# AIBluefisher/DAGSfM

Hardware: NVIDIA B200
Metric: image_pairs_verified_per_s (higher is better)
Workload: dtype f64 (verification) / u8 x u8 -> s32 exact (matching)

## Files before the change

### dagsfm_b200/csrc/verify_api.cu

```cuda
#include <cuda_runtime.h>

#include <algorithm>
#include <cstdio>
#include <cstdlib>
#include <cstring>
#include <vector>

#include "../../include/dagsfm_b200.h"
#include "common_host.h"
#include "verify_common.cuh"
#include "verify_multiple.h"

using namespace b2;

struct b2_verifier {
  int device = 0;
  int n_sm = 148;
  cudaStream_t stream = nullptr;
  int32_t n_images = 0;
  b2_camera* d_cams = nullptr;
  int64_t* d_img_off = nullptr;
  double* d_xy = nullptr;
  double* d_nxy = nullptr;
  int64_t n_pts_total = 0;
// ... 90 lines not shown
  }
  B2_CUDA(cudaMemsetAsync(v->d_err, 0, sizeof(int), s));
  VerifyArgs a;
  a.cams = v->d_cams;
  a.img_off = v->d_img_off;
  a.n_images = v->n_images;
  a.xy = (const double2*)v->d_xy;
  a.nxy = (const double2*)v->d_nxy;
  a.matches = matches;
  a.opt = *opt;
  a.inlier_out = inl;
  a.scratch = v->d_scratch;
  a.scratch_stride = stride;
  a.m_cap = m_cap;
  a.max_workers = blocks * wpb;
  a.work_counter = v->d_counter;
  a.state = (VerifyPairState*)v->d_state;
  a.masks = v->d_masks;
  a.mask_stride = std::max<int64_t>(max_span, 1);
  a.err = v->d_err;
  a.prof = nullptr;
  unsigned long long* d_prof = nullptr;
  if (getenv("B2_VERIFY_PROFILE")) {
    B2_CUDA(cudaMalloc(&d_prof, 8 * sizeof(unsigned long long)));
    B2_CUDA(cudaMemsetAsync(d_prof, 0, 8 * sizeof(unsigned long long), s));
    a.prof = d_prof;
  }
  B2_CUDA(cudaEventRecord(v->ev0, s));
  for (int64_t b = 0; b < n_batches; ++b) {
    const int64_t p0 = b * kStageBatch, p1 = std::min(n_pairs, p0 + kStageBatch);
    a.n_pairs = p1 - p0;
    a.pairs = pairs + 2 * p0;
    a.match_off = off + p0;
    a.seeds = seeds + p0;
    a.results = results + p0;
    a.mask_base = bound[(size_t)b];
    B2_CUDA(cudaMemsetAsync(v->d_counter, 0, 4 * sizeof(unsigned long long), s));
    B2_CUDA(launch_verify_pairs(a, v->n_sm, s));
    count_launches(4);
  }
  B2_CUDA(cudaEventRecord(v->ev1, s));
  count_launches(1);
  int err = 0;
  B2_CUDA(cudaMemcpyAsync(&err, v->d_err, sizeof(int), cudaMemcpyDeviceToHost, s));
  B2_CUDA(cudaStreamSynchronize(s));
  float ms = 0;
  B2_CUDA(cudaEventElapsedTime(&ms, v->ev0, v->ev1));
  v->last_kernel_s = ms * 1e-3;
  if (d_prof) {
    unsigned long long hp[8];
    cudaMemcpy(hp, d_prof, sizeof hp, cudaMemcpyDeviceToHost);
    cudaFree(d_prof);
    fprintf(stderr, "[b2 verify profile] warp-cycles: sample %.3g solve %.3g score %.3g lo %.3g | E %.3g F %.3g H %.3g T %.3g | kernel %.3f s\n",
            (double)hp[0], (double)hp[1], (double)hp[2], (double)hp[3], (double)hp[4], (double)hp[5], (double)hp[6], (double)hp[7], v->last_kernel_s);
  }
  if (err == 2) return set_error(B2_ERR_CUDA, "sampler FIFO exhausted inside one batch of trials (more than 256 raw draws)");
  if (err) return set_error(B2_ERR_INVALID, "pair references an image outside the store");
  return B2_OK;
}

int stage(b2_verifier* v, size_t bytes) {
  if (bytes <= v->stage_bytes) return B2_OK;
  if (v->d_stage) cudaFree(v->d_stage);
  v->d_stage = nullptr;
  v->stage_bytes = 0;
  B2_CUDA(cudaMalloc(&v->d_stage, bytes));
  v->stage_bytes = bytes;
  return B2_OK;
}

}

extern "C" {

void b2_two_view_default_options(b2_two_view_options* o) {
  if (!o) return;
  o->min_num_inliers = 15;
// ... 259 lines not shown
  if (n_pairs == 0) return check_options(opt);
  const int64_t total = match_offsets[n_pairs];
  if (total < 0 || (total > 0 && (!matches || !inlier_matches))) return set_error(B2_ERR_INVALID, "NULL match buffers");
  auto round = [&](int64_t na, const int64_t* ids, const int64_t* off, const uint32_t* m, const uint32_t* sd,
                   b2_two_view_result* res, uint32_t* inl) -> int {
    std::vector<uint32_t> pr((size_t)na * 2);
    for (int64_t k = 0; k < na; ++k) {
      pr[2 * k] = pairs[2 * ids[k]];
      pr[2 * k + 1] = pairs[2 * ids[k] + 1];
    }
    return b2_verify_pairs(v, na, pr.data(), off, m, opt, sd, res, inl);
  };
  return estimate_multiple(n_pairs, match_offsets, matches, seeds, multiple_ignore_watermark != 0, round, results,
                           inlier_matches);
}

int b2_score_models(b2_verifier* v, int32_t type, int32_t n, const double* xy1, const double* xy2, int32_t n_models,
                    const double* models, double max_residual, int32_t* counts, double* sums, uint8_t* masks) {
  if (!v || n < 0 || n_models < 0 || type < 0 || type > 3) return set_error(B2_ERR_INVALID, "bad argument");
  if (n_models == 0) return B2_OK;
  B2_CUDA(cudaSetDevice(v->device));
  auto al = [](size_t b) { return (b + 255) / 256 * 256; };
  const size_t bp = al((size_t)std::max(n, 1) * 16), bm = al((size_t)n_models * 72), bc = al((size_t)n_models * 4),
               bs = al((size_t)n_models * 8), bk = al((size_t)n_models * std::max(n, 1));
  B2_TRY(stage(v, 2 * bp + bm + bc + bs + bk));
  uint8_t* p = (uint8_t*)v->d_stage;
  double* d1 = (double*)p; p += bp;
  double* d2 = (double*)p; p += bp;
  double* dm = (double*)p; p += bm;
  int* dc = (int*)p; p += bc;
  double* ds = (double*)p; p += bs;
  uint8_t* dk = p;
  cudaStream_t s = v->stream;
  if (n > 0) {
    B2_CUDA(cudaMemcpyAsync(d1, xy1, (size_t)n * 16, cudaMemcpyHostToDevice, s));
    B2_CUDA(cudaMemcpyAsync(d2, xy2, (size_t)n * 16, cudaMemcpyHostToDevice, s));
  }
  B2_CUDA(cudaMemcpyAsync(dm, models, (size_t)n_models * 72, cudaMemcpyHostToDevice, s));
  B2_CUDA(launch_score_models(type, n, d1, d2, n_models, dm, max_residual, dc, ds, dk, s));
  count_launches(1);
  B2_CUDA(cudaMemcpyAsync(counts, dc, (size_t)n_models * 4, cudaMemcpyDeviceToHost, s));
  B2_CUDA(cudaMemcpyAsync(sums, ds, (size_t)n_models * 8, cudaMemcpyDeviceToHost, s));
  if (n > 0 && masks) B2_CUDA(cudaMemcpyAsync(masks, dk, (size_t)n_models * n, cudaMemcpyDeviceToHost, s));
  B2_CUDA(cudaStreamSynchronize(s));
  return B2_OK;
}

int b2_verify_debug_sample_stream(b2_verifier* v, uint32_t seed, int32_t total, int32_t k, int32_t n_trials,
                                  int32_t* out) {
  if (!v || !out || total < k || k < 1 || k > 8 || n_trials < 0) return set_error(B2_ERR_INVALID, "bad argument");
  B2_CUDA(cudaSetDevice(v->device));
  B2_TRY(stage(v, (size_t)total * 4 + (size_t)std::max(n_trials, 1) * k * 4 + 512));
  uint32_t* d_idx = (uint32_t*)v->d_stage;
  int* d_out = (int*)((uint8_t*)v->d_stage + ((size_t)total * 4 + 255) / 256 * 256);
  B2_CUDA(launch_debug_sample_stream(seed, total, k, n_trials, d_idx, d_out, v->stream));
  B2_CUDA(cudaMemcpyAsync(out, d_out, (size_t)n_trials * k * 4, cudaMemcpyDeviceToHost, v->stream));
  B2_CUDA(cudaStreamSynchronize(v->stream));
  return B2_OK;
}

int b2_verify_debug_solve(b2_verifier* v, int32_t type, int32_t n, const double* xy1, const double* xy2,
                          double* models_out, int32_t* n_models) {
// ... 36 lines not shown
```

### dagsfm_b200/csrc/verify_common.cuh

```cuda
#pragma once
#include <cuda_runtime.h>

#include <cstdint>

#include "../../include/dagsfm_b200.h"

namespace b2 {

enum { EST_E5 = 0, EST_F7 = 1, EST_H4 = 2, EST_T2 = 3 };
__host__ __device__ inline int min_samples(int t) { return t == EST_E5 ? 5 : t == EST_F7 ? 7 : t == EST_H4 ? 4 : 1; }
__host__ __device__ inline int local_min_samples(int t) { return t == EST_E5 ? 5 : t == EST_F7 ? 8 : t == EST_H4 ? 4 : 1; }

struct VerifyRansacReport {
  int32_t success, num_inliers;
  long long num_trials;
  double model[9];
};
struct VerifyPairState {
  uint32_t mt[624];
  uint32_t ring[256];
  uint32_t mti, w, r, pad;
  VerifyRansacReport report[3];
};

// ... 4 lines not shown
  const double2* xy;
  const double2* nxy;
  int64_t n_pairs;
  const uint32_t* pairs;
  const int64_t* match_off;
  const uint32_t* matches;
  const uint32_t* seeds;
  b2_two_view_options opt;
  b2_two_view_result* results;
  uint32_t* inlier_out;
  uint8_t* scratch;
  size_t scratch_stride;
  int32_t m_cap;
  int32_t max_workers;
  unsigned long long* work_counter;
  VerifyPairState* state;
  uint8_t* masks;
  int64_t mask_stride, mask_base;
  int* err;
  unsigned long long* prof;
};

size_t verify_scratch_stride(int m_cap);
int verify_warps_per_block();
int verify_blocks_per_sm();
cudaError_t launch_normalize_points(const b2_camera* cams, const int64_t* img_off, int n_images, const double* xy,
                                    double* nxy, int64_t n_total, cudaStream_t s);
cudaError_t launch_verify_pairs(const VerifyArgs& a, int n_sm, cudaStream_t s);
cudaError_t launch_relative_pose(const b2_camera* cams, const int64_t* img_off, int n_images, const double* nxy,
                                 int64_t n_pairs, const uint32_t* pairs, const int64_t* match_off,
                                 const b2_two_view_result* results, const uint32_t* inliers, b2_relative_pose* poses,
                                 double* angles, int* err, int n_sm, cudaStream_t s);
cudaError_t launch_score_models(int type, int n, const double* p1, const double* p2, int n_models, const double* models,
                                double max_res, int* counts, double* sums, uint8_t* masks, cudaStream_t s);
cudaError_t launch_debug_sample_stream(uint32_t seed, int total, int k, int n_trials, uint32_t* idx, int* out,
                                       cudaStream_t s);
cudaError_t launch_debug_solve(int type, int n, const double* p1, const double* p2, double* G, uint32_t* inl,
                               double* models, int* n_models, cudaStream_t s);

}
```

### dagsfm_b200/csrc/verify_kernel.cu

```cuda
#include <cuda_runtime.h>

#include <cfloat>
#include <cstdint>
#include <algorithm>
#include <cstdlib>
#include <cstring>

#include "../../include/dagsfm_b200.h"
#include "verify_common.cuh"
#include "verify_solvers.cuh"
#include "camera_models.cuh"

namespace b2 {
namespace vf {

constexpr unsigned kFull = 0xffffffffu;
constexpr int kWarpsPerBlock = 8;
constexpr int kThreads = 32 * kWarpsPerBlock;
using LaneView = View<1>;

constexpr int kIdxSmem = 2048;
struct WarpShared {
  double V[81];
  double R[81];
  double sig[9];
  uint32_t mt[624];
  uint32_t ring[256];
  uint16_t idx16[kIdxSmem];
  uint32_t samp[32][8];
  uint32_t pos_after[32];
  int cnt[320];
  uint16_t flat[320];
  uint16_t off[34];
  uint16_t lo_ids[12];
  int lo_cnt[12];
  int nm[32];
  int lo_nm;
  uint32_t mti, w, r;
  uint32_t r0, overflow;
};

static_assert(sizeof(WarpShared) % 8 == 0, "WarpShared must keep doubles aligned");
constexpr size_t kDynSmemBytes = sizeof(WarpShared) * kWarpsPerBlock;

__device__ inline void mt_seed(WarpShared& s, uint32_t seed) {
  s.mt[0] = seed;
  for (int i = 1; i < 624; ++i) s.mt[i] = 1812433253u * (s.mt[i - 1] ^ (s.mt[i - 1] >> 30)) + (uint32_t)i;
  s.mti = 624;
  s.w = 0;
  s.r = 0;
  s.r0 = 0;
}
__device__ inline uint32_t mt_next(WarpShared& s) {
  if (s.mti >= 624) {
    for (int k = 0; k < 624; ++k) {
      const uint32_t y = (s.mt[k] & 0x80000000u) | (s.mt[(k + 1) % 624] & 0x7fffffffu);
      s.mt[k] = s.mt[(k + 397) % 624] ^ (y >> 1) ^ ((y & 1u) ? 0x9908b0dfu : 0u);
    }
    s.mti = 0;
  }
// ... 57 lines not shown
    if ((uint32_t)lane < c) {
      uint32_t y = s.mt[mti + lane];
      y ^= (y >> 11);
      y ^= (y << 7) & 0x9d2c5680u;
      y ^= (y << 15) & 0xefc60000u;
      y ^= (y >> 18);
      s.ring[(w + lane) & 255u] = y;
    }
    __syncwarp();
    if (lane == 0) { s.mti = mti + c; s.w = w + c; }
    __syncwarp();
  }
}

__device__ __forceinline__ double sampson(const double* E, double x1_0, double x1_1, double x2_0, double x2_1) {
  const double Ex1_0 = E[0] * x1_0 + E[1] * x1_1 + E[2];
  const double Ex1_1 = E[3] * x1_0 + E[4] * x1_1 + E[5];
  const double Ex1_2 = E[6] * x1_0 + E[7] * x1_1 + E[8];
  const double Etx2_0 = E[0] * x2_0 + E[3] * x2_1 + E[6];
  const double Etx2_1 = E[1] * x2_0 + E[4] * x2_1 + E[7];
  const double x2tEx1 = x2_0 * Ex1_0 + x2_1 * Ex1_1 + Ex1_2;
  return x2tEx1 * x2tEx1 / (Ex1_0 * Ex1_0 + Ex1_1 * Ex1_1 + Etx2_0 * Etx2_0 + Etx2_1 * Etx2_1);
}
__device__ __forceinline__ double transfer(const double* H, double s_0, double s_1, double d_0, double d_1) {
  const double pd_0 = H[0] * s_0 + H[1] * s_1 + H[2];
  const double pd_1 = H[3] * s_0 + H[4] * s_1 + H[5];
  const double pd_2 = H[6] * s_0 + H[7] * s_1 + H[8];
  const double inv_pd_2 = 1.0 / pd_2;
  const double dd_0 = d_0 - pd_0 * inv_pd_2;
  const double dd_1 = d_1 - pd_1 * inv_pd_2;
  return dd_0 * dd_0 + dd_1 * dd_1;
}
__device__ __forceinline__ double translation_res(const double* T, double a0, double a1, double b0, double b1) {
  const double e0 = (b0 - a0) - T[0], e1 = (b1 - a1) - T[1];
  return e0 * e0 + e1 * e1;
}
template <int TYPE>
__device__ __forceinline__ double residual_t(const double* M, double2 a, double2 b) {
  if (TYPE == EST_H4) return transfer(M, a.x, a.y, b.x, b.y);
  if (TYPE == EST_T2) return translation_res(M, a.x, a.y, b.x, b.y);
  return sampson(M, a.x, a.y, b.x, b.y);
}

constexpr int kGroup = 4;

template <int TYPE, int G>
__device__ __noinline__ void score_group(const double2* __restrict__ P1, const double2* __restrict__ P2, int M,
                                         const double* __restrict__ models, const uint16_t* ids, int n, double max_res,
                                         int lane, int* cnt_out) {
  double m[G][9];
#pragma unroll
  for (int u = 0; u < G; ++u) {
    const int id = ids[u < n ? u : n - 1];
    const double* src = models + (id / 10) * 90 + (id % 10) * 9;
#pragma unroll
// ... 5 lines not shown
  int i = lane;
  double2 a = P1[i < M ? i : 0], b = P2[i < M ? i : 0];
  for (; i < M; i += 32) {
    const int nx = i + 32 < M ? i + 32 : i;
    const double2 an = P1[nx], bn = P2[nx];
#pragma unroll
    for (int u = 0; u < G; ++u) c[u] += (residual_t<TYPE>(m[u], a, b) <= max_res) ? 1 : 0;
    a = an;
    b = bn;
  }
#pragma unroll
  for (int u = 0; u < G; ++u) {
#pragma unroll
    for (int o = 16; o > 0; o >>= 1) c[u] += __shfl_xor_sync(kFull, c[u], o);
  }
  if (lane == 0) {
#pragma unroll
    for (int u = 0; u < G; ++u)
      if (u < n) cnt_out[ids[u]] = c[u];
  }
  __syncwarp();
}
template <int TYPE> struct ResidualOf { static constexpr int value = (TYPE == EST_H4 || TYPE == EST_T2) ? TYPE : EST_F7; };

template <int TYPE>
__device__ __noinline__ int score_count(const double2* P1, const double2* P2, int M, const double* model, double max_res,
                           int lane) {
  int cnt = 0;
  for (int i0 = 0; i0 < M; i0 += 32) {
    const int i = i0 + lane;
    bool in = false;
    if (i < M) in = residual_t<TYPE>(model, P1[i], P2[i]) <= max_res;
    cnt += __popc(__ballot_sync(kFull, in));
  }
  return cnt;
}
template <int TYPE>
__device__ __noinline__ double score_sum(const double2* P1, const double2* P2, int M, const double* model, double max_res,
                            int lane, uint8_t* mask_out) {
  double sum = 0;
  for (int i0 = 0; i0 < M; i0 += 32) {
    const int i = i0 + lane;
    bool in = false;
    double r = 0;
    if (i < M) {
      r = residual_t<TYPE>(model, P1[i], P2[i]);
// ... 285 lines not shown
    for (int k = lane; k < N; k += 32) {
      const double2 s = apply_T(T1, P1[inl[k]]), d = apply_T(T2, P2[inl[k]]);
      const int j = N + k;
      G[0 * (size_t)ld + k] = -s.x; G[1 * (size_t)ld + k] = -s.y; G[2 * (size_t)ld + k] = -1;
      G[3 * (size_t)ld + k] = 0; G[4 * (size_t)ld + k] = 0; G[5 * (size_t)ld + k] = 0;
      G[6 * (size_t)ld + k] = s.x * d.x; G[7 * (size_t)ld + k] = s.y * d.x; G[8 * (size_t)ld + k] = d.x;
      G[0 * (size_t)ld + j] = 0; G[1 * (size_t)ld + j] = 0; G[2 * (size_t)ld + j] = 0;
      G[3 * (size_t)ld + j] = -s.x; G[4 * (size_t)ld + j] = -s.y; G[5 * (size_t)ld + j] = -1;
      G[6 * (size_t)ld + j] = s.x * d.y; G[7 * (size_t)ld + j] = s.y * d.y; G[8 * (size_t)ld + j] = d.y;
    }
  }
  __syncwarp();
  warp_svd9(G, rows, ld, sh, lane);
  if (lane == 0) {
    double nv[9];
    for (int k = 0; k < 9; ++k) nv[k] = sh.V[k * 9 + 8];
    if (type == EST_F7) finish_f8(nv, T1, T2, models);
    else finish_h(nv, T1, T2, models);
  }
  __syncwarp();
  return 1;
}

struct RansacResult {
  bool success;
  int num_inliers;
  double residual_sum;
  long long num_trials;
  double model[9];
};

struct Scratch {
  double2 *px1, *px2;
  double2 *ip1, *ip2;
  uint32_t* idx;
  uint32_t* inl;
  double* G;
  int ld;
  double* models;
  double* lomodels;
  uint8_t* tmask;
  unsigned long long* prof;
};

template <int type, int GS>
__device__ __noinline__ void ransac_warp(const double2* P1, const double2* P2, int M, double max_error,
                            double min_inlier_ratio, double confidence, long long min_num_trials,
                            long long max_num_trials_opt, WarpShared& sh, double* sig_sh, const Scratch& sc,
                            uint8_t* mask_out, RansacResult* out, int lane, LaneView ws) {
  const int kmin = min_samples(type), klo = local_min_samples(type);
  out->success = false;
  out->num_trials = 0;
  out->num_inliers = 0;
  out->residual_sum = DBL_MAX;
  for (int k = 0; k < 9; ++k) out->model[k] = 0.0;
  unsigned long long max_trials = (unsigned long long)max_num_trials_opt;
  {
    const unsigned long long dyn = compute_num_trials((unsigned long long)(min_inlier_ratio * 100000.0), 100000ull, confidence, kmin);
    if (dyn < max_trials) max_trials = dyn;
  }
  if (M < kmin) return;
  const double max_residual = max_error * max_error;
  int best_count = 0;
  double best_sum = DBL_MAX;
  double best_model[9];
  for (int k = 0; k < 9; ++k) best_model[k] = 0.0;
  bool abort = false;
  if (lane < 12) sh.lo_ids[lane] = (uint16_t)lane;
  const bool idx_sm = M <= kIdxSmem;
  if (idx_sm) for (int i = lane; i < M; i += 32) sh.idx16[i] = (uint16_t)i;
  else for (int i = lane; i < M; i += 32) sc.idx[i] = (uint32_t)i;
  __syncwarp();
  unsigned long long dyn_max = max_trials;
  unsigned long long t0 = 0;
  unsigned long long num_trials = 0;
  bool ended = false;
  while (t0 < max_trials) {
    if (abort) {
      num_trials = t0 + 1;
      ended = true;
      break;
    }
    const int nb = (int)((max_trials - t0) < 32ull ? (max_trials - t0) : 32ull);
    const long long c0 = clock64();
    {
      const uint32_t need = (uint32_t)(nb * kmin);
      ring_fill_warp(sh, need, lane);
      const uint32_t r = sh.r;
      bool suspect = false;
      for (uint32_t d = lane; d < need; d += 32) {
        const uint32_t i = d % (uint32_t)kmin, j = d / (uint32_t)kmin;
        const uint32_t range = (uint32_t)M - i;
        const uint64_t product = (uint64_t)sh.ring[(r + d) & 255u] * (uint64_t)range;
        suspect |= (uint32_t)product < range;
        sh.samp[j][i] = (uint32_t)(product >> 32) + i;
// ... 40 lines not shown
        else {
          for (int k = 0; k < 9; ++k) mm[k] = 0.0;
          mm[0] = b[0] / 1.0 - a[0] / 1.0;
          mm[1] = b[1] / 1.0 - a[1] / 1.0;
          nm = 1;
        }
        for (int k = 0; k < 9 * nm; ++k) mymodels[k] = mm[k];
      }
      sh.nm[lane] = nm;
      int incl = nm;
#pragma unroll
      for (int d = 1; d < 32; d <<= 1) {
        const int t = __shfl_up_sync(kFull, incl, d);
        if (lane >= d) incl += t;
      }
      const int first = incl - nm;
      sh.off[lane] = (uint16_t)first;
      if (lane == 31) sh.off[32] = (uint16_t)incl;
      for (int mi = 0; mi < nm; ++mi) sh.flat[first + mi] = (uint16_t)(lane * 10 + mi);
    }
    __syncwarp();
    const long long c2 = clock64();
    long long lo_cycles = 0;
    for (int j = 0; j < nb; ++j) {
      const unsigned long long trial = t0 + j;
      if (abort) {
        num_trials = trial + 1;
        ended = true;
        if (lane == 0) sh.r = sh.pos_after[j - 1];
        break;
      }
      if ((j & 7) == 0) {
        const int g1 = sh.off[min(j + 8, 32)];
        for (int g = sh.off[j]; g < g1; g += GS)
          score_group<ResidualOf<type>::value, GS>(P1, P2, M, sc.models, sh.flat + g, min(GS, g1 - g), max_residual, lane, sh.cnt);
      }
      const int nm = sh.nm[j];
      for (int mi = 0; mi < nm; ++mi) {
        const int cnt = sh.cnt[j * 10 + mi];
        bool better = cnt > best_count;
        double sum = 0;
        double model[9];
        if (cnt >= best_count) {
          for (int k = 0; k < 9; ++k) model[k] = sc.models[(size_t)j * 90 + 9 * mi + k];
          sum = score_sum<ResidualOf<type>::value>(P1, P2, M, model, max_residual, lane, sc.tmask);
          sum = __shfl_sync(kFull, sum, 0);
          if (cnt == best_count) better = sum < best_sum;
        }
        if (better) {
          best_count = cnt;
          best_sum = sum;
          for (int k = 0; k < 9; ++k) best_model[k] = model[k];
          if (cnt > kmin && cnt >= klo) {
            __syncwarp();
            int N = 0;
            for (int i0 = 0; i0 < M; i0 += 32) {
              const int i = i0 + lane;
              const bool in = (i < M) && sc.tmask[i];
              const unsigned bm = __ballot_sync(kFull, in);
              if (in) sc.inl[N + __popc(bm & ((1u << lane) - 1))] = (uint32_t)i;
              N += __popc(bm);
            }
            __syncwarp();
            const long long cl0 = clock64();
            const int nlm = local_estimate<type>(P1, P2, sc.inl, N, sc.G, sc.ld, sh, sig_sh, sc.lomodels, lane);
            lo_cycles += clock64() - cl0;
            for (int g = 0; g < nlm; g += GS)
              score_group<ResidualOf<type>::value, GS>(P1, P2, M, sc.lomodels, sh.lo_ids + g, min(GS, nlm - g), max_residual, lane,
                                                       sh.lo_cnt);
            for (int li = 0; li < nlm; ++li) {
              double lm[9];
              for (int k = 0; k < 9; ++k) lm[k] = sc.lomodels[9 * li + k];
              const int lc = sh.lo_cnt[li];
              bool lbetter = lc > best_count;
              double lsum = 0;
              if (lc >= best_count) {
                lsum = score_sum<ResidualOf<type>::value>(P1, P2, M, lm, max_residual, lane, nullptr);
                lsum = __shfl_sync(kFull, lsum, 0);
                if (lc == best_count) lbetter = lsum < best_sum;
              }
              if (lbetter) {
                best_count = lc;
                best_sum = lsum;
                for (int k = 0; k < 9; ++k) best_model[k] = lm[k];
              }
            }
          }
          dyn_max = compute_num_trials((unsigned long long)best_count, (unsigned long long)M, confidence, kmin);
        }
        if (trial >= dyn_max && trial >= (unsigned long long)min_num_trials) {
          abort = true;
          break;
        }
      }
    }
    if (sc.prof && lane == 0) {
      const long long c3 = clock64();
      atomicAdd(sc.prof + 0, (unsigned long long)(c1 - c0));
      atomicAdd(sc.prof + 1, (unsigned long long)(c2 - c1));
      atomicAdd(sc.prof + 2, (unsigned long long)(c3 - c2 - lo_cycles));
      atomicAdd(sc.prof + 3, (unsigned long long)lo_cycles);
      atomicAdd(sc.prof + 4 + (type == EST_E5 ? 0 : type == EST_F7 ? 1 : type == EST_H4 ? 2 : 3), (unsigned long long)(c3 - c0));
    }
    if (ended) break;
    t0 += nb;
    __syncwarp();
  }
  if (!ended) num_trials = max_trials;
  out->num_trials = (long long)num_trials;
  out->num_inliers = best_count;
  out->residual_sum = best_sum;
  for (int k = 0; k < 9; ++k) out->model[k] = best_model[k];
  if (best_count < kmin) return;
  out->success = true;
  score_sum<ResidualOf<type>::value>(P1, P2, M, best_model, max_residual, lane, mask_out);
  __syncwarp();
}

__device__ inline void simple_radial_distortion(double k, double u, double v, double* du, double* dv) {
  const double u2 = u * u, v2 = v * v, r2 = u2 + v2, radial = k * r2;
  *du = u * radial;
  *dv = v * radial;
}
__device__ inline double2 image_to_world(const b2_camera& c, double2 p) {
  double u, v;
// ... 58 lines not shown
__device__ __forceinline__ bool in_box(double2 p, double minx, double maxx, double miny, double maxy) {
  return p.x >= minx && p.x <= maxx && p.y >= miny && p.y <= maxy;
}

__device__ __forceinline__ void prng_save(const WarpShared& sh, VerifyPairState& st, int lane) {
  for (int i = lane; i < 624; i += 32) st.mt[i] = sh.mt[i];
  for (int i = lane; i < 256; i += 32) st.ring[i] = sh.ring[i];
  if (lane == 0) { st.mti = sh.mti; st.w = sh.w; st.r = sh.r; }
}
__device__ __forceinline__ void prng_load(WarpShared& sh, const VerifyPairState& st, int lane) {
  for (int i = lane; i < 624; i += 32) sh.mt[i] = st.mt[i];
  for (int i = lane; i < 256; i += 32) sh.ring[i] = st.ring[i];
  if (lane == 0) { sh.mti = st.mti; sh.w = st.w; sh.r = st.r; sh.r0 = st.r; }
}
__device__ __forceinline__ void report_store(VerifyRansacReport& d, const RansacResult& r, int lane) {
  if (lane == 0) {
    d.success = r.success ? 1 : 0;
    d.num_inliers = r.num_inliers;
    d.num_trials = r.num_trials;
    for (int k = 0; k < 9; ++k) d.model[k] = r.model[k];
  }
}

__host__ __device__ constexpr int stage_group(int bps) { return bps >= 2 ? 2 : kGroup; }

template <int STAGE, int BPS>
__global__ void __launch_bounds__(kThreads, BPS) verify_stage_kernel(VerifyArgs A) {
  extern __shared__ double warp_sh[];
  double lane_work[kLaneWorkDoubles];
  const LaneView ws{lane_work};
  const int lane = threadIdx.x & 31, wib = threadIdx.x >> 5;
  WarpShared& sh = reinterpret_cast<WarpShared*>(warp_sh)[wib];
  double* sig_sh = sh.sig;
  const int worker = blockIdx.x * (int)(blockDim.x >> 5) + wib;
  Scratch sc;
  {
    uint8_t* base = A.scratch + (size_t)worker * A.scratch_stride;
    const size_t mc = (size_t)A.m_cap;
    sc.px1 = (double2*)base; base += mc * 16;
    sc.px2 = (double2*)base; base += mc * 16;
    sc.ip1 = (double2*)base; base += mc * 16;
    sc.ip2 = (double2*)base; base += mc * 16;
    sc.G = (double*)base; base += mc * 2 * 9 * 8;
    sc.ld = (int)(2 * mc);
    sc.models = (double*)base; base += 32 * 90 * 8;
    sc.lomodels = (double*)base; base += 90 * 8;
    sc.idx = (uint32_t*)base; base += mc * 4;
    sc.inl = (uint32_t*)base; base += mc * 4;
    sc.tmask = base;
    sc.prof = A.prof;
  }
  const b2_two_view_options& o = A.opt;
  constexpr int GS = stage_group(BPS);
  if (lane == 0) sh.overflow = 0;
  __syncwarp();
  for (;;) {
    long long p = 0;
    if (lane == 0) p = (long long)atomicAdd(A.work_counter + STAGE, 1ull);
    p = __shfl_sync(kFull, p, 0);
    if (p >= A.n_pairs) break;
    const uint32_t i1 = A.pairs[2 * p], i2 = A.pairs[2 * p + 1];
    const int64_t moff = A.match_off[p];
    const int M = (int)(A.match_off[p + 1] - moff);
    const bool invalid = i1 >= (uint32_t)A.n_images || i2 >= (uint32_t)A.n_images || M > A.m_cap;
    const bool skip = invalid || (unsigned long long)M < (unsigned long long)o.min_num_inliers;
    VerifyPairState& st = A.state[p];
    uint8_t* const masks = A.masks + (moff - A.mask_base);
    if (STAGE < 3) {
      if (skip) continue;
      const b2_camera c1 = A.cams[i1], c2 = A.cams[i2];
      const bool calibrated = c1.has_prior_focal_length && c2.has_prior_focal_length;
      const uint32_t* mt = A.matches + 2 * moff;
      const int64_t o1 = A.img_off[i1], o2 = A.img_off[i2];
      const double2* src = (STAGE == 0) ? A.nxy : A.xy;
      if (STAGE == 0) {
        if (lane == 0) mt_seed(sh, A.seeds[p]);
      } else {
        prng_load(sh, st, lane);
      }
      const bool run = STAGE != 0 || calibrated;
      if (run)
        for (int i = lane; i < M; i += 32) {
          sc.px1[i] = src[o1 + mt[2 * i]];
          sc.px2[i] = src[o2 + mt[2 * i + 1]];
        }
      __syncwarp();
      RansacResult R;
      R.success = false; R.num_inliers = 0; R.num_trials = 0; R.residual_sum = 0;
      for (int k = 0; k < 9; ++k) R.model[k] = 0.0;
      if (run) {
        double err = o.max_error;
        if (STAGE == 0) err = (image_to_world_threshold(c1, o.max_error) + image_to_world_threshold(c2, o.max_error)) / 2;
        constexpr int TYPE = STAGE == 0 ? EST_E5 : STAGE == 1 ? EST_F7 : EST_H4;
        ransac_warp<TYPE, GS>(sc.px1, sc.px2, M, err, o.min_inlier_ratio, o.confidence, o.min_num_trials, o.max_num_trials,
                              sh, sig_sh, sc, masks + (size_t)STAGE * A.mask_stride, &R, lane, ws);
      }
      report_store(st.report[STAGE], R, lane);
      __syncwarp();
      prng_save(sh, st, lane);
      if (lane == 0 && sh.overflow) atomicExch(A.err, 2);
      __syncwarp();
      continue;
    }
    b2_two_view_result res;
    res.config = 0;
    res.n_inliers = 0;
    res.E_num_inliers = res.F_num_inliers = res.H_num_inliers = 0;
    res.E_num_trials = res.F_num_trials = res.H_num_trials = 0;
// ... 88 lines not shown
        if (o.detect_watermark) {
          const double ratio = (double)nb_border / (double)num_inliers;
          if (!(ratio < o.watermark_min_inlier_ratio)) {
            prng_load(sh, st, lane);
            __syncwarp();
            RansacResult T;
            ransac_warp<EST_T2, kGroup>(sc.ip1, sc.ip2, (int)num_inliers, o.max_error, o.watermark_min_inlier_ratio,
                                        o.confidence, o.min_num_trials, o.max_num_trials, sh, sig_sh, sc, sc.tmask, &T, lane, ws);
            const double inlier_ratio = (double)T.num_inliers / (double)num_inliers;
            if (inlier_ratio >= o.watermark_min_inlier_ratio) res.config = 7;
          }
        }
      }
    }
    if (lane == 0) {
      A.results[p] = res;
      if (sh.overflow) atomicExch(A.err, 2);
    }
    __syncwarp();
  }
}


__global__ void score_models_kernel(int type, int n, const double2* P1, const double2* P2, int n_models,
                                    const double* models, double max_res, int* counts, double* sums, uint8_t* masks) {
  const int lane = threadIdx.x & 31;
  const int w = (blockIdx.x * blockDim.x + threadIdx.x) >> 5;
  if (w >= n_models) return;
  double model[9];
  for (int k = 0; k < 9; ++k) model[k] = models[9 * w + k];
  int c;
  double s;
  uint8_t* mk = masks + (size_t)w * n;
  if (type == EST_H4) { c = score_count<EST_H4>(P1, P2, n, model, max_res, lane); s = score_sum<EST_H4>(P1, P2, n, model, max_res, lane, mk); }
  else if (type == EST_T2) { c = score_count<EST_T2>(P1, P2, n, model, max_res, lane); s = score_sum<EST_T2>(P1, P2, n, model, max_res, lane, mk); }
  else { c = score_count<EST_F7>(P1, P2, n, model, max_res, lane); s = score_sum<EST_F7>(P1, P2, n, model, max_res, lane, mk); }
  s = __shfl_sync(kFull, s, 0);
  if (lane == 0) {
    counts[w] = c;
    sums[w] = s;
  }
}

__global__ void debug_sample_stream_kernel(uint32_t seed, int total, int k, int n_trials, uint32_t* idx, int* out) {
  __shared__ WarpShared sh;
  if (threadIdx.x == 0) {
    mt_seed(sh, seed);
    for (int i = 0; i < total; ++i) idx[i] = i;
    for (int t = 0; t < n_trials; ++t) {
      for (uint32_t i = 0; i < (uint32_t)k; ++i) {
        const uint32_t j = uniform_u32(sh, i, (uint32_t)(total - 1));
        const uint32_t a = idx[i], b = idx[j];
        idx[i] = b;
        idx[j] = a;
      }
      for (int i = 0; i < k; ++i) out[t * k + i] = (int)idx[i];
    }
// ... 21 lines not shown
    __syncwarp();
    const int nm = type == EST_E5 ? local_estimate<EST_E5>(P1, P2, inl, n, G, 2 * n, sh, sig, models, lane)
                 : type == EST_F7 ? local_estimate<EST_F7>(P1, P2, inl, n, G, 2 * n, sh, sig, models, lane)
                                  : local_estimate<EST_H4>(P1, P2, inl, n, G, 2 * n, sh, sig, models, lane);
    if (lane == 0) *n_models = nm;
    return;
  }
  {
    double a[14], b[14], mm[90];
    for (int i = 0; i < n; ++i) { a[2 * i] = P1[i].x; a[2 * i + 1] = P1[i].y; b[2 * i] = P2[i].x; b[2 * i + 1] = P2[i].y; }
    int nm = 0;
    if (type == EST_E5) nm = solve_e5(ws, a, b, mm);
    else if (type == EST_F7) nm = solve_f7(ws, a, b, mm);
    else nm = solve_h4(ws, a, b, mm);
    if (lane == 0) {
      for (int k = 0; k < 9 * nm; ++k) models[k] = mm[k];
      *n_models = nm;
    }
  }
}

}

size_t verify_scratch_stride(int m_cap) {
  const size_t mc = (size_t)m_cap;
  size_t b = mc * 16 * 4 + mc * 2 * 9 * 8 + 32 * 90 * 8 + 90 * 8 + mc * 4 * 2 + mc;
  return (b + 255) / 256 * 256;
}
void verify_stage_shapes(int bps[3]) {
  bps[0] = 1; bps[1] = 1; bps[2] = 1;
  const char* e = getenv("B2_VERIFY_BPS");
  if (e && strlen(e) == 3)
    for (int k = 0; k < 3; ++k) bps[k] = e[k] == '2' ? 2 : 1;
}
int verify_warps_per_block() { return vf::kWarpsPerBlock; }
int verify_blocks_per_sm() {
  int b[3];
  verify_stage_shapes(b);
  return std::max(b[0], std::max(b[1], b[2]));
}

cudaError_t launch_normalize_points(const b2_camera* cams, const int64_t* img_off, int n_images, const double* xy,
                                    double* nxy, int64_t n_total, cudaStream_t s) {
  if (n_total == 0) return cudaSuccess;
  vf::normalize_points_kernel<<<(unsigned)((n_total + 127) / 128), 128, 0, s>>>(
      cams, img_off, n_images, (const double2*)xy, (double2*)nxy, n_total);
  return cudaGetLastError();
}
template <int STAGE, int BPS>
// ... 1 lines not shown
  const size_t dyn = vf::kDynSmemBytes;
  cudaError_t e = cudaFuncSetAttribute(vf::verify_stage_kernel<STAGE, BPS>, cudaFuncAttributeMaxDynamicSharedMemorySize, (int)dyn);
  if (e != cudaSuccess) return e;
  int blocks = n_sm * BPS;
  blocks = (int)std::min<int64_t>(blocks, (a.n_pairs + vf::kWarpsPerBlock - 1) / vf::kWarpsPerBlock);
  blocks = std::min(blocks, a.max_workers / vf::kWarpsPerBlock);
  if (blocks < 1) blocks = 1;
  vf::verify_stage_kernel<STAGE, BPS><<<blocks, vf::kThreads, dyn, s>>>(a);
  return cudaGetLastError();
}
cudaError_t launch_verify_pairs(const VerifyArgs& a, int n_sm, cudaStream_t s) {
  int bps[3];
  verify_stage_shapes(bps);
  cudaError_t e;
  e = bps[0] == 2 ? launch_stage<0, 2>(a, n_sm, s) : launch_stage<0, 1>(a, n_sm, s);
  if (e != cudaSuccess) return e;
  e = bps[1] == 2 ? launch_stage<1, 2>(a, n_sm, s) : launch_stage<1, 1>(a, n_sm, s);
  if (e != cudaSuccess) return e;
  e = bps[2] == 2 ? launch_stage<2, 2>(a, n_sm, s) : launch_stage<2, 1>(a, n_sm, s);
  if (e != cudaSuccess) return e;
  return launch_stage<3, 1>(a, n_sm, s);
}
cudaError_t launch_score_models(int type, int n, const double* p1, const double* p2, int n_models, const double* models,
                                double max_res, int* counts, double* sums, uint8_t* masks, cudaStream_t s) {
  if (n_models == 0) return cudaSuccess;
  vf::score_models_kernel<<<(n_models + 3) / 4, 128, 0, s>>>(type, n, (const double2*)p1, (const double2*)p2, n_models,
                                                              models, max_res, counts, sums, masks);
  return cudaGetLastError();
}
cudaError_t launch_debug_sample_stream(uint32_t seed, int total, int k, int n_trials, uint32_t* idx, int* out,
                                       cudaStream_t s) {
  vf::debug_sample_stream_kernel<<<1, 32, 0, s>>>(seed, total, k, n_trials, idx, out);
  return cudaGetLastError();
}
cudaError_t launch_debug_solve(int type, int n, const double* p1, const double* p2, double* G, uint32_t* inl,
                               double* models, int* n_models, cudaStream_t s) {
  const size_t dyn = vf::kDynSmemBytes;
  cudaError_t e = cudaFuncSetAttribute(vf::debug_solve_kernel, cudaFuncAttributeMaxDynamicSharedMemorySize, (int)dyn);
  if (e != cudaSuccess) return e;
  vf::debug_solve_kernel<<<1, vf::kThreads, dyn, s>>>(type, n, (const double2*)p1, (const double2*)p2, G, inl, models,
                                                     n_models);
  return cudaGetLastError();
}

}
```

Measured before the change: 63010.

## Add certified FP32 homography inlier filter with FP64 fallback and early exit

Homography RANSAC scoring now first evaluates each point against each model in FP32 using prepacked float points and per-pair magnitude bounds. A certified error bound decides whether the FP32 sign is trustworthy, and only uncertain points fall back to the exact FP64 transfer error. The H stage also gets a larger model group size and an early break when no model in the group can beat the current best count. This aims to cut FP64 work on the B200, at the cost of extra scratch memory, a float point copy per pair, and register pressure from the wider group.

```diff
diff --git a/dagsfm_b200/csrc/verify_api.cu b/dagsfm_b200/csrc/verify_api.cu
--- a/dagsfm_b200/csrc/verify_api.cu
+++ b/dagsfm_b200/csrc/verify_api.cu
@@ -136,8 +136,8 @@
   a.prof = nullptr;
   unsigned long long* d_prof = nullptr;
   if (getenv("B2_VERIFY_PROFILE")) {
-    B2_CUDA(cudaMalloc(&d_prof, 8 * sizeof(unsigned long long)));
-    B2_CUDA(cudaMemsetAsync(d_prof, 0, 8 * sizeof(unsigned long long), s));
+    B2_CUDA(cudaMalloc(&d_prof, kVerifyProfCounters * sizeof(unsigned long long)));
+    B2_CUDA(cudaMemsetAsync(d_prof, 0, kVerifyProfCounters * sizeof(unsigned long long), s));
     a.prof = d_prof;
   }
   B2_CUDA(cudaEventRecord(v->ev0, s));
@@ -162,11 +162,17 @@
   B2_CUDA(cudaEventElapsedTime(&ms, v->ev0, v->ev1));
   v->last_kernel_s = ms * 1e-3;
   if (d_prof) {
-    unsigned long long hp[8];
+    unsigned long long hp[kVerifyProfCounters];
     cudaMemcpy(hp, d_prof, sizeof hp, cudaMemcpyDeviceToHost);
     cudaFree(d_prof);
-    fprintf(stderr, "[b2 verify profile] warp-cycles: sample %.3g solve %.3g score %.3g lo %.3g | E %.3g F %.3g H %.3g T %.3g | kernel %.3f s\n",
-            (double)hp[0], (double)hp[1], (double)hp[2], (double)hp[3], (double)hp[4], (double)hp[5], (double)hp[6], (double)hp[7], v->last_kernel_s);
+    fprintf(stderr, "[b2 verify profile] warp-cycles (sample solve count score lo):");
+    for (int e = 0; e < 4; ++e) {
+      const unsigned long long* q = hp + 5 * e;
+      fprintf(stderr, " | %c %.3g %.3g %.3g %.3g %.3g = %.3g", "EFHT"[e], (double)q[0], (double)q[1], (double)q[2], (double)q[3],
+              (double)q[4], (double)(q[0] + q[1] + q[2] + q[3] + q[4]));
+    }
+    fprintf(stderr, " | H transfer evaluations %.4g, FP64 fallbacks %.4g (%.3g%%) | kernel %.3f s\n", (double)hp[20],
+            (double)hp[21], hp[20] ? 100.0 * (double)hp[21] / (double)hp[20] : 0.0, v->last_kernel_s);
   }
   if (err == 2) return set_error(B2_ERR_CUDA, "sampler FIFO exhausted inside one batch of trials (more than 256 raw draws)");
   if (err) return set_error(B2_ERR_INVALID, "pair references an image outside the store");
@@ -472,22 +478,23 @@
   B2_CUDA(cudaSetDevice(v->device));
   auto al = [](size_t b) { return (b + 255) / 256 * 256; };
   const size_t bp = al((size_t)std::max(n, 1) * 16), bm = al((size_t)n_models * 72), bc = al((size_t)n_models * 4),
-               bs = al((size_t)n_models * 8), bk = al((size_t)n_models * std::max(n, 1));
-  B2_TRY(stage(v, 2 * bp + bm + bc + bs + bk));
+               bs = al((size_t)n_models * 8), bk = al((size_t)n_models * std::max(n, 1)), bh = al(verify_h_points_bytes(n));
+  B2_TRY(stage(v, 2 * bp + bm + bc + bs + bk + bh));
   uint8_t* p = (uint8_t*)v->d_stage;
   double* d1 = (double*)p; p += bp;
   double* d2 = (double*)p; p += bp;
   double* dm = (double*)p; p += bm;
   int* dc = (int*)p; p += bc;
   double* ds = (double*)p; p += bs;
-  uint8_t* dk = p;
+  uint8_t* dk = p; p += bk;
+  void* dh = p;
   cudaStream_t s = v->stream;
   if (n > 0) {
     B2_CUDA(cudaMemcpyAsync(d1, xy1, (size_t)n * 16, cudaMemcpyHostToDevice, s));
     B2_CUDA(cudaMemcpyAsync(d2, xy2, (size_t)n * 16, cudaMemcpyHostToDevice, s));
   }
   B2_CUDA(cudaMemcpyAsync(dm, models, (size_t)n_models * 72, cudaMemcpyHostToDevice, s));
-  B2_CUDA(launch_score_models(type, n, d1, d2, n_models, dm, max_residual, dc, ds, dk, s));
+  B2_CUDA(launch_score_models(type, n, d1, d2, n_models, dm, max_residual, dc, ds, dk, dh, s));
   count_launches(1);
   B2_CUDA(cudaMemcpyAsync(counts, dc, (size_t)n_models * 4, cudaMemcpyDeviceToHost, s));
   B2_CUDA(cudaMemcpyAsync(sums, ds, (size_t)n_models * 8, cudaMemcpyDeviceToHost, s));
diff --git a/dagsfm_b200/csrc/verify_common.cuh b/dagsfm_b200/csrc/verify_common.cuh
--- a/dagsfm_b200/csrc/verify_common.cuh
+++ b/dagsfm_b200/csrc/verify_common.cuh
@@ -50,6 +50,8 @@
 };
 
 size_t verify_scratch_stride(int m_cap);
+constexpr int kVerifyProfCounters = 22;
+size_t verify_h_points_bytes(int n);
 int verify_warps_per_block();
 int verify_blocks_per_sm();
 cudaError_t launch_normalize_points(const b2_camera* cams, const int64_t* img_off, int n_images, const double* xy,
@@ -60,7 +62,7 @@
                                  const b2_two_view_result* results, const uint32_t* inliers, b2_relative_pose* poses,
                                  double* angles, int* err, int n_sm, cudaStream_t s);
 cudaError_t launch_score_models(int type, int n, const double* p1, const double* p2, int n_models, const double* models,
-                                double max_res, int* counts, double* sums, uint8_t* masks, cudaStream_t s);
+                                double max_res, int* counts, double* sums, uint8_t* masks, void* hscratch, cudaStream_t s);
 cudaError_t launch_debug_sample_stream(uint32_t seed, int total, int k, int n_trials, uint32_t* idx, int* out,
                                        cudaStream_t s);
 cudaError_t launch_debug_solve(int type, int n, const double* p1, const double* p2, double* G, uint32_t* inl,
diff --git a/dagsfm_b200/csrc/verify_hfilter.cuh b/dagsfm_b200/csrc/verify_hfilter.cuh
--- /dev/null
+++ b/dagsfm_b200/csrc/verify_hfilter.cuh
@@ -0,0 +1,75 @@
+#pragma once
+
+namespace b2 {
+namespace vf {
+
+__device__ __forceinline__ double transfer(const double* H, double s_0, double s_1, double d_0, double d_1) {
+  const double pd_0 = H[0] * s_0 + H[1] * s_1 + H[2];
+  const double pd_1 = H[3] * s_0 + H[4] * s_1 + H[5];
+  const double pd_2 = H[6] * s_0 + H[7] * s_1 + H[8];
+  const double inv_pd_2 = 1.0 / pd_2;
+  const double dd_0 = d_0 - pd_0 * inv_pd_2;
+  const double dd_1 = d_1 - pd_1 * inv_pd_2;
+  return dd_0 * dd_0 + dd_1 * dd_1;
+}
+
+struct HPairBounds {
+  float x, y, d;
+  int ok;
+};
+struct alignas(16) HPoint {
+  float s0, s1, d0, d1;
+};
+struct HFilter {
+  float h[9];
+  float ce, c0, dw, t;
+};
+constexpr float kHKappa = 0x1p-19f;
+
+__device__ __forceinline__ float h_f32(double v, bool& ok) {
+  const bool in = fabs(v) <= 0x1p30;
+  ok = ok && in;
+  return in ? (float)v : 0.0f;
+}
+
+__device__ inline HFilter h_filter_make(const double* H, const HPairBounds& b, double t) {
+  HFilter f;
+  bool ok = b.ok != 0;
+  for (int k = 0; k < 9; ++k) ok = ok && fabs(H[k]) <= 0x1p60;
+  double A[3];
+  for (int k = 0; k < 3; ++k)
+    A[k] = (fabs(H[3 * k]) * (double)b.x + fabs(H[3 * k + 1]) * (double)b.y + fabs(H[3 * k + 2])) * (1.0 + 0x1p-20);
+  const double Amax = A[0] > A[1] ? A[0] : A[1], W = A[2];
+  ok = ok && A[0] <= 0x1p40 && A[1] <= 0x1p40 && W <= 0x1p40 && (double)b.d * W <= 0x1p40 &&
+       (t == 0.0 || (t >= 0x1p-60 && t <= 0x1p40));
+  for (int k = 0; k < 9; ++k) f.h[k] = ok ? (float)H[k] : 0.0f;
+  if (!ok) {
+    f.ce = 0.0f;
+    f.c0 = INFINITY;
+    f.dw = 0.0f;
+    f.t = 0.0f;
+    return f;
+  }
+  const double delta = 0x1p-20 * ((double)b.d * W + Amax) + 0x1p-100;
+  f.ce = (float)(2.0 * delta);
+  f.c0 = (float)(2.0 * delta * delta + 0x1p-18 * t * W * W + 0x1p-120);
+  f.dw = (float)(0x1p-19 * W + 0x1p-90);
+  f.t = (float)t;
+  return f;
+}
+
+__device__ __forceinline__ bool h_filter_eval(const HFilter& f, float s0, float s1, float d0, float d1, bool& inlier) {
+  const float p0 = fmaf(f.h[0], s0, fmaf(f.h[1], s1, f.h[2]));
+  const float p1 = fmaf(f.h[3], s0, fmaf(f.h[4], s1, f.h[5]));
+  const float w = fmaf(f.h[6], s0, fmaf(f.h[7], s1, f.h[8]));
+  const float e0 = fmaf(d0, w, -p0), e1 = fmaf(d1, w, -p1);
+  const float n = fmaf(e1, e1, e0 * e0);
+  const float tw = f.t * (w * w);
+  const float L = n - tw;
+  const float E = fmaf(kHKappa, n + tw, fmaf(f.ce, fabsf(e0) + fabsf(e1), f.c0));
+  inlier = L < 0.0f;
+  return fabsf(L) > E && fabsf(w) > f.dw;
+}
+
+}
+}
diff --git a/dagsfm_b200/csrc/verify_kernel.cu b/dagsfm_b200/csrc/verify_kernel.cu
--- a/dagsfm_b200/csrc/verify_kernel.cu
+++ b/dagsfm_b200/csrc/verify_kernel.cu
@@ -9,6 +9,7 @@
 #include "../../include/dagsfm_b200.h"
 #include "verify_common.cuh"
 #include "verify_solvers.cuh"
+#include "verify_hfilter.cuh"
 #include "camera_models.cuh"
 
 namespace b2 {
@@ -36,6 +37,7 @@
   int lo_cnt[12];
   int nm[32];
   int lo_nm;
+  HPairBounds hb;
   uint32_t mti, w, r;
   uint32_t r0, overflow;
 };
@@ -139,15 +141,6 @@
   const double x2tEx1 = x2_0 * Ex1_0 + x2_1 * Ex1_1 + Ex1_2;
   return x2tEx1 * x2tEx1 / (Ex1_0 * Ex1_0 + Ex1_1 * Ex1_1 + Etx2_0 * Etx2_0 + Etx2_1 * Etx2_1);
 }
-__device__ __forceinline__ double transfer(const double* H, double s_0, double s_1, double d_0, double d_1) {
-  const double pd_0 = H[0] * s_0 + H[1] * s_1 + H[2];
-  const double pd_1 = H[3] * s_0 + H[4] * s_1 + H[5];
-  const double pd_2 = H[6] * s_0 + H[7] * s_1 + H[8];
-  const double inv_pd_2 = 1.0 / pd_2;
-  const double dd_0 = d_0 - pd_0 * inv_pd_2;
-  const double dd_1 = d_1 - pd_1 * inv_pd_2;
-  return dd_0 * dd_0 + dd_1 * dd_1;
-}
 __device__ __forceinline__ double translation_res(const double* T, double a0, double a1, double b0, double b1) {
   const double e0 = (b0 - a0) - T[0], e1 = (b1 - a1) - T[1];
   return e0 * e0 + e1 * e1;
@@ -199,6 +192,81 @@
   __syncwarp();
 }
 template <int TYPE> struct ResidualOf { static constexpr int value = (TYPE == EST_H4 || TYPE == EST_T2) ? TYPE : EST_F7; };
+
+__device__ __forceinline__ int warp_sum(int v) {
+#pragma unroll
+  for (int o = 16; o > 0; o >>= 1) v += __shfl_xor_sync(kFull, v, o);
+  return v;
+}
+template <int G>
+__device__ __noinline__ void score_group_h(const HPoint* __restrict__ PF, const double2* __restrict__ P1,
+                                           const double2* __restrict__ P2, int M, const HPairBounds hb,
+                                           const double* __restrict__ models, const uint16_t* ids, int n, double max_res,
+                                           int best_count, int lane, int* cnt_out, unsigned long long* prof) {
+  HFilter f[G];
+#pragma unroll
+  for (int u = 0; u < G; ++u) {
+    const int id = ids[u < n ? u : n - 1];
+    f[u] = h_filter_make(models + (id / 10) * 90 + (id % 10) * 9, hb, max_res);
+  }
+  const unsigned live = (1u << n) - 1u;
+  int c[G];
+#pragma unroll
+  for (int u = 0; u < G; ++u) c[u] = 0;
+  int fallbacks = 0;
+  int i0 = 0;
+  HPoint q = PF[lane < M ? lane : 0];
+  for (; i0 < M; i0 += 32) {
+    const int i = i0 + lane;
+    const HPoint qn = PF[i + 32 < M ? i + 32 : (i < M ? i : 0)];
+    if (i < M) {
+      unsigned unc = 0;
+#pragma unroll
+      for (int u = 0; u < G; ++u) {
+        bool in;
+        const bool certain = h_filter_eval(f[u], q.s0, q.s1, q.d0, q.d1, in);
+        c[u] += (certain && in) ? 1 : 0;
+        unc |= certain ? 0u : (1u << u);
+      }
+      unc &= live;
+      if (unc) {
+        const double2 a = P1[i], b = P2[i];
+        fallbacks += __popc(unc);
+#pragma unroll
+        for (int u = 0; u < G; ++u) {
+          if (unc & (1u << u)) {
+            const int id = ids[u];
+            c[u] += transfer(models + (id / 10) * 90 + (id % 10) * 9, a.x, a.y, b.x, b.y) <= max_res ? 1 : 0;
+          }
+        }
+      }
+    }
+    q = qn;
+    const int remaining = M - (i0 + 32);
+    if ((i0 & 127) == 96 && remaining < best_count) {
+      bool hopeless = true;
+#pragma unroll
+      for (int u = 0; u < G; ++u) hopeless &= warp_sum(c[u]) + remaining < best_count;
+      if (hopeless) {
+        i0 += 32;
+        break;
+      }
+    }
+  }
+#pragma unroll
+  for (int u = 0; u < G; ++u) c[u] = warp_sum(c[u]);
+  if (prof) fallbacks = warp_sum(fallbacks);
+  if (lane == 0) {
+#pragma unroll
+    for (int u = 0; u < G; ++u)
+      if (u < n) cnt_out[ids[u]] = c[u];
+    if (prof) {
+      atomicAdd(prof + 0, (unsigned long long)n * (unsigned long long)min(i0, M));
+      atomicAdd(prof + 1, (unsigned long long)fallbacks);
+    }
+  }
+  __syncwarp();
+}
 
 template <int TYPE>
 __device__ __noinline__ int score_count(const double2* P1, const double2* P2, int M, const double* model, double max_res,
@@ -530,6 +598,23 @@
   return 1;
 }
 
+__device__ __forceinline__ HPoint h_point_f32(double2 a, double2 b, float& mx, float& my, float& md, bool& fin) {
+  const HPoint q = HPoint{h_f32(a.x, fin), h_f32(a.y, fin), h_f32(b.x, fin), h_f32(b.y, fin)};
+  mx = fmaxf(mx, fabsf(q.s0));
+  my = fmaxf(my, fabsf(q.s1));
+  md = fmaxf(md, fmaxf(fabsf(q.d0), fabsf(q.d1)));
+  return q;
+}
+__device__ inline HPairBounds h_pair_bounds_warp(float mx, float my, float md, bool fin) {
+#pragma unroll
+  for (int o = 16; o > 0; o >>= 1) {
+    mx = fmaxf(mx, __shfl_xor_sync(kFull, mx, o));
+    my = fmaxf(my, __shfl_xor_sync(kFull, my, o));
+    md = fmaxf(md, __shfl_xor_sync(kFull, md, o));
+  }
+  return HPairBounds{mx, my, md, __any_sync(kFull, !fin) ? 0 : 1};
+}
+
 struct RansacResult {
   bool success;
   int num_inliers;
@@ -541,6 +626,7 @@
 struct Scratch {
   double2 *px1, *px2;
   double2 *ip1, *ip2;
+  HPoint* pf;
   uint32_t* idx;
   uint32_t* inl;
   double* G;
@@ -550,6 +636,9 @@
   uint8_t* tmask;
   unsigned long long* prof;
 };
+enum { kProfSample, kProfSolve, kProfCount, kProfScore, kProfLo, kProfPhases };
+constexpr int kProfEvals = 4 * kProfPhases, kProfFallbacks = kProfEvals + 1;
+static_assert(kProfFallbacks + 1 == kVerifyProfCounters, "verify_api.cu sizes the counters");
 
 template <int type, int GS>
 __device__ __noinline__ void ransac_warp(const double2* P1, const double2* P2, int M, double max_error,
@@ -579,6 +668,16 @@
   if (idx_sm) for (int i = lane; i < M; i += 32) sh.idx16[i] = (uint16_t)i;
   else for (int i = lane; i < M; i += 32) sc.idx[i] = (uint32_t)i;
   __syncwarp();
+  long long count_cycles = 0;
+  auto count = [&](const double* models, const uint16_t* ids, int n, int* cnt_out) {
+    const long long cc0 = clock64();
+    if constexpr (type == EST_H4)
+      score_group_h<GS>(sc.pf, P1, P2, M, sh.hb, models, ids, n, max_residual, best_count, lane, cnt_out,
+                        sc.prof ? sc.prof + kProfEvals : nullptr);
+    else
+      score_group<ResidualOf<type>::value, GS>(P1, P2, M, models, ids, n, max_residual, lane, cnt_out);
+    count_cycles += clock64() - cc0;
+  };
   unsigned long long dyn_max = max_trials;
   unsigned long long t0 = 0;
   unsigned long long num_trials = 0;
@@ -665,6 +764,7 @@
     __syncwarp();
     const long long c2 = clock64();
     long long lo_cycles = 0;
+    count_cycles = 0;
     for (int j = 0; j < nb; ++j) {
       const unsigned long long trial = t0 + j;
       if (abort) {
@@ -675,8 +775,7 @@
       }
       if ((j & 7) == 0) {
         const int g1 = sh.off[min(j + 8, 32)];
-        for (int g = sh.off[j]; g < g1; g += GS)
-          score_group<ResidualOf<type>::value, GS>(P1, P2, M, sc.models, sh.flat + g, min(GS, g1 - g), max_residual, lane, sh.cnt);
+        for (int g = sh.off[j]; g < g1; g += GS) count(sc.models, sh.flat + g, min(GS, g1 - g), sh.cnt);
       }
       const int nm = sh.nm[j];
       for (int mi = 0; mi < nm; ++mi) {
@@ -708,9 +807,7 @@
             const long long cl0 = clock64();
             const int nlm = local_estimate<type>(P1, P2, sc.inl, N, sc.G, sc.ld, sh, sig_sh, sc.lomodels, lane);
             lo_cycles += clock64() - cl0;
-            for (int g = 0; g < nlm; g += GS)
-              score_group<ResidualOf<type>::value, GS>(P1, P2, M, sc.lomodels, sh.lo_ids + g, min(GS, nlm - g), max_residual, lane,
-                                                       sh.lo_cnt);
+            for (int g = 0; g < nlm; g += GS) count(sc.lomodels, sh.lo_ids + g, min(GS, nlm - g), sh.lo_cnt);
             for (int li = 0; li < nlm; ++li) {
               double lm[9];
               for (int k = 0; k < 9; ++k) lm[k] = sc.lomodels[9 * li + k];
@@ -739,11 +836,12 @@
     }
     if (sc.prof && lane == 0) {
       const long long c3 = clock64();
-      atomicAdd(sc.prof + 0, (unsigned long long)(c1 - c0));
-      atomicAdd(sc.prof + 1, (unsigned long long)(c2 - c1));
-      atomicAdd(sc.prof + 2, (unsigned long long)(c3 - c2 - lo_cycles));
-      atomicAdd(sc.prof + 3, (unsigned long long)lo_cycles);
-      atomicAdd(sc.prof + 4 + (type == EST_E5 ? 0 : type == EST_F7 ? 1 : type == EST_H4 ? 2 : 3), (unsigned long long)(c3 - c0));
+      unsigned long long* pe = sc.prof + kProfPhases * (type == EST_E5 ? 0 : type == EST_F7 ? 1 : type == EST_H4 ? 2 : 3);
+      atomicAdd(pe + kProfSample, (unsigned long long)(c1 - c0));
+      atomicAdd(pe + kProfSolve, (unsigned long long)(c2 - c1));
+      atomicAdd(pe + kProfCount, (unsigned long long)count_cycles);
+      atomicAdd(pe + kProfScore, (unsigned long long)(c3 - c2 - lo_cycles - count_cycles));
+      atomicAdd(pe + kProfLo, (unsigned long long)lo_cycles);
     }
     if (ended) break;
     t0 += nb;
@@ -848,7 +946,9 @@
   }
 }
 
-__host__ __device__ constexpr int stage_group(int bps) { return bps >= 2 ? 2 : kGroup; }
+__host__ __device__ constexpr int stage_group(int stage, int bps) {
+  return stage == 2 ? (bps >= 2 ? 4 : 8) : (bps >= 2 ? 2 : kGroup);
+}
 
 template <int STAGE, int BPS>
 __global__ void __launch_bounds__(kThreads, BPS) verify_stage_kernel(VerifyArgs A) {
@@ -867,6 +967,7 @@
     sc.px2 = (double2*)base; base += mc * 16;
     sc.ip1 = (double2*)base; base += mc * 16;
     sc.ip2 = (double2*)base; base += mc * 16;
+    sc.pf = (HPoint*)base; base += mc * 16;
     sc.G = (double*)base; base += mc * 2 * 9 * 8;
     sc.ld = (int)(2 * mc);
     sc.models = (double*)base; base += 32 * 90 * 8;
@@ -877,7 +978,7 @@
     sc.prof = A.prof;
   }
   const b2_two_view_options& o = A.opt;
-  constexpr int GS = stage_group(BPS);
+  constexpr int GS = stage_group(STAGE, BPS);
   if (lane == 0) sh.overflow = 0;
   __syncwarp();
   for (;;) {
@@ -905,11 +1006,20 @@
         prng_load(sh, st, lane);
       }
       const bool run = STAGE != 0 || calibrated;
-      if (run)
+      if (run) {
+        float mx = 0.0f, my = 0.0f, md = 0.0f;
+        bool fin = true;
         for (int i = lane; i < M; i += 32) {
-          sc.px1[i] = src[o1 + mt[2 * i]];
-          sc.px2[i] = src[o2 + mt[2 * i + 1]];
-        }
+          const double2 a = src[o1 + mt[2 * i]], b = src[o2 + mt[2 * i + 1]];
+          sc.px1[i] = a;
+          sc.px2[i] = b;
+          if (STAGE == 2) sc.pf[i] = h_point_f32(a, b, mx, my, md, fin);
+        }
+        if (STAGE == 2) {
+          const HPairBounds hb = h_pair_bounds_warp(mx, my, md, fin);
+          if (lane == 0) sh.hb = hb;
+        }
+      }
       __syncwarp();
       RansacResult R;
       R.success = false; R.num_inliers = 0; R.num_trials = 0; R.residual_sum = 0;
@@ -1044,8 +1154,17 @@
 }
 
 
-__global__ void score_models_kernel(int type, int n, const double2* P1, const double2* P2, int n_models,
-                                    const double* models, double max_res, int* counts, double* sums, uint8_t* masks) {
+__global__ void h_points_kernel(int n, const double2* P1, const double2* P2, HPoint* pf, HPairBounds* hb) {
+  const int lane = threadIdx.x & 31;
+  float mx = 0.0f, my = 0.0f, md = 0.0f;
+  bool fin = true;
+  for (int i = lane; i < n; i += 32) pf[i] = h_point_f32(P1[i], P2[i], mx, my, md, fin);
+  const HPairBounds b = h_pair_bounds_warp(mx, my, md, fin);
+  if (lane == 0) *hb = b;
+}
+__global__ void score_models_kernel(int type, int n, const double2* P1, const double2* P2, const HPoint* pf,
+                                    const HPairBounds* hb, int n_models, const double* models, double max_res, int* counts,
+                                    double* sums, uint8_t* masks) {
   const int lane = threadIdx.x & 31;
   const int w = (blockIdx.x * blockDim.x + threadIdx.x) >> 5;
   if (w >= n_models) return;
@@ -1054,7 +1173,16 @@
   int c;
   double s;
   uint8_t* mk = masks + (size_t)w * n;
-  if (type == EST_H4) { c = score_count<EST_H4>(P1, P2, n, model, max_res, lane); s = score_sum<EST_H4>(P1, P2, n, model, max_res, lane, mk); }
+  if (type == EST_H4) {
+    if (n > 0) {
+      const uint16_t id0 = 0;
+      score_group_h<stage_group(2, 1)>(pf, P1, P2, n, *hb, models + 9 * w, &id0, 1, max_res, 0, lane, counts + w, nullptr);
+    } else if (lane == 0) {
+      counts[w] = 0;
+    }
+    c = counts[w];
+    s = score_sum<EST_H4>(P1, P2, n, model, max_res, lane, mk);
+  }
   else if (type == EST_T2) { c = score_count<EST_T2>(P1, P2, n, model, max_res, lane); s = score_sum<EST_T2>(P1, P2, n, model, max_res, lane, mk); }
   else { c = score_count<EST_F7>(P1, P2, n, model, max_res, lane); s = score_sum<EST_F7>(P1, P2, n, model, max_res, lane, mk); }
   s = __shfl_sync(kFull, s, 0);
@@ -1122,9 +1250,10 @@
 
 }
 
+size_t verify_h_points_bytes(int n) { return (size_t)n * sizeof(vf::HPoint) + sizeof(vf::HPairBounds); }
 size_t verify_scratch_stride(int m_cap) {
   const size_t mc = (size_t)m_cap;
-  size_t b = mc * 16 * 4 + mc * 2 * 9 * 8 + 32 * 90 * 8 + 90 * 8 + mc * 4 * 2 + mc;
+  size_t b = mc * 16 * 5 + mc * 2 * 9 * 8 + 32 * 90 * 8 + 90 * 8 + mc * 4 * 2 + mc;
   return (b + 255) / 256 * 256;
 }
 void verify_stage_shapes(int bps[3]) {
@@ -1172,10 +1301,17 @@
   return launch_stage<3, 1>(a, n_sm, s);
 }
 cudaError_t launch_score_models(int type, int n, const double* p1, const double* p2, int n_models, const double* models,
-                                double max_res, int* counts, double* sums, uint8_t* masks, cudaStream_t s) {
+                                double max_res, int* counts, double* sums, uint8_t* masks, void* hscratch, cudaStream_t s) {
   if (n_models == 0) return cudaSuccess;
-  vf::score_models_kernel<<<(n_models + 3) / 4, 128, 0, s>>>(type, n, (const double2*)p1, (const double2*)p2, n_models,
-                                                              models, max_res, counts, sums, masks);
+  vf::HPoint* pf = (vf::HPoint*)hscratch;
+  vf::HPairBounds* hb = (vf::HPairBounds*)(pf + n);
+  if (type == EST_H4) {
+    vf::h_points_kernel<<<1, 32, 0, s>>>(n, (const double2*)p1, (const double2*)p2, pf, hb);
+    const cudaError_t e = cudaGetLastError();
+    if (e != cudaSuccess) return e;
+  }
+  vf::score_models_kernel<<<(n_models + 3) / 4, 128, 0, s>>>(type, n, (const double2*)p1, (const double2*)p2, pf, hb,
+                                                              n_models, models, max_res, counts, sums, masks);
   return cudaGetLastError();
 }
 cudaError_t launch_debug_sample_stream(uint32_t seed, int total, int k, int n_trials, uint32_t* idx, int* out,
```

Result: slower. 52060, median of 6 (-17.4%).
